# Kinetica-jl/Kinetica.jl

Hardware: AMD Instinct MI355X
Metric: RHS evals/sec (batched sweep) + wall-clock per solve_network, 10k-species CRN (higher is better)
Workload: dtype f64; 1 GPU; synthetic CRN 10000 species / 50000 reactions (seed 12345), batched RHS sweep, B=4096 states per GPU with per-state Arrhenius k (500-1200 K); states_per_gpu=4096, parallelism=replicas x1 (no data-path collective)

## Files before the change

### kinetica_jl_amd/csrc/capi.cpp

```cpp
#include "../../include/kinetica_hip.h"

#include <algorithm>
#include <cmath>
#include <memory>
#include <mutex>
#include <numeric>
#include <string>
#include <cstring>
#include <thread>
#include <vector>

#include "handle.hpp"
#include "lu.hpp"
#include "resident_setup.hpp"
#include "solver.hpp"
#include "solver_kernels.hpp"

using namespace kin;

static thread_local std::string g_create_err;

void kin_network::flush_pending_T(hipStream_t s) {
  if (!k_pending) return;
  launch_arrhenius(host.R, Ea.p, A.p, has_kmax, k_max, t_mult, T_pending, k.p, s);
// ... 1 lines not shown
}

void kin_network::rhs_dev(const double* d_u, double* d_du) {
  if (k_pending) { launch_rates_T(host.R, pending_at(), k.p, d_u, x0.p, x1.p, rate.p, stream); k_pending = false; }
  else launch_rates(host.R, k.p, d_u, x0.p, x1.p, rate.p, stream);
  launch_segsum(rhs_plan.view(), SEG_COEF_SET, rate.p, d_du, SegExtra{}, stream);
}

void kin_network::sweep_dev(int64_t B, const double* d_u, const double* d_k, double* d_du, hipStream_t s) {
  if (!d_k) flush_pending_T(s);
  if (host.N >= 65535) {
    for (int64_t b = 0; b < B; b++) {
      launch_rates(host.R, d_k ? d_k + b * host.R : k.p, d_u + b * host.N, x0.p, x1.p, rate.p, s);
      launch_segsum(rhs_plan.view(), SEG_COEF_SET, rate.p, d_du + b * host.N, SegExtra{}, s);
    }
  } else if (host.big_H > 0) {
    big_scratch.alloc((size_t)std::min<int64_t>(B, n_cu) * (size_t)(host.N - host.big_H + host.n_pairs()));
    launch_sweep_big(n_cu, host.N, host.R, host.n_pairs(), B, host.pairs_adjacent, host.big_H, (int32_t)host.big_tail_ptr.size() - 1,
                     big_rec8.p, big_rec.p, big_expl.p, (int32_t)host.big_expl.size(), sweep_k.p, big_spec.p, big_tptr.p, big_tent.p,
                     big_scratch.p, d_u, d_k, k.p, d_du, host.big_tail_by_species, s);
  } else
    launch_sweep(n_cu, host.N, host.R, host.n_pairs(), B, host.pairs_adjacent, host.pairs_block, sweep_rec.p, sweep_k.p,
                 host.pair_rec64.empty() ? nullptr : sweep_rec64.p, sweep_copy.p, (int)host.sweep_copy_species.size(),
                 host.gen_rec8.empty() ? nullptr : gen_rec8.p, gen_expl.p, (int)host.gen_expl.size(), d_u, d_k, k.p, d_du, s);
}

void kin_network::jac_dev(const double* d_u, double* d_vals) {
  if (k_pending) { launch_drates_T(host.R, pending_at(), k.p, d_u, x0.p, x1.p, dr.p, stream); k_pending = false; }
  else launch_drates(host.R, k.p, d_u, x0.p, x1.p, dr.p, stream);
  launch_segsum(jac_plan.view(), SEG_COEF_SET, dr.p, d_vals, SegExtra{}, stream);
}

#define KIN_TRY(h) try { if (h) KIN_HIP(hipSetDevice((h)->device));
#define KIN_CATCH(h)                                                        \
  }                                                                         \
  catch (const KinError& e) {                                               \
    if (h) (h)->err = e.what(); else g_create_err = e.what();               \
    return e.code;                                                          \
  }                                                                         \
  catch (const std::exception& e) {                                         \
    if (h) (h)->err = e.what(); else g_create_err = e.what();               \
    return KIN_ERR_DEVICE;                                                  \
  }                                                                         \
  return KIN_OK;

static void require(bool c, int code, const char* msg) {
  if (!c) throw KinError(code, msg);
// ... 23 lines not shown

int kin_network_create(int64_t n_species, int64_t n_reactions, const int64_t* reac_ptr, const int64_t* reac_idx,
                       const int64_t* reac_sto, const int64_t* prod_ptr, const int64_t* prod_idx,
                       const int64_t* prod_sto, int index_base, kin_network** out) {
  kin_network* h = nullptr;
  if (!out) { g_create_err = "out is null"; return KIN_ERR_INVALID_ARG; }
  *out = nullptr;
  try {
    NetworkHost H = compile_network(n_species, n_reactions, reac_ptr, reac_idx, reac_sto, prod_ptr, prod_idx,
                                    prod_sto, index_base);
    int ndev = 0;
    if (hipGetDeviceCount(&ndev) != hipSuccess || ndev == 0)
      throw KinError(ERR_DEVICE, "no HIP device available (libkinetica_hip has no CPU fallback)");
    h = new kin_network();
    h->host = std::move(H);
    KIN_HIP(hipGetDevice(&h->device));
    KIN_HIP(hipDeviceGetAttribute(&h->n_cu, hipDeviceAttributeMultiprocessorCount, h->device));
    KIN_HIP(hipStreamCreateWithFlags(&h->stream, hipStreamNonBlocking));
    const NetworkHost& N = h->host;
    hipStream_t s = h->stream;
    h->x0.upload(N.x0, s); h->x1.upload(N.x1, s);
    h->sp_ptr.upload(N.sp_ptr, s); h->sp_rxn.upload(N.sp_rxn, s); h->sp_coef.upload(N.sp_coef, s);
    if (N.N < 65535) { h->sweep_rec.upload(N.pair_rec, s); h->sweep_k.upload(N.pair_k, s); }
    if (!N.gen_rec8.empty()) { h->gen_rec8.upload(N.gen_rec8, s); h->gen_expl.upload(N.gen_expl, s); }
    if (!N.pair_rec64.empty()) { h->sweep_rec64.upload(N.pair_rec64, s); h->sweep_copy.upload(N.sweep_copy_species, s); }
    if (N.big_H > 0) {
      h->big_rec.upload(N.big_rec, s); h->big_rec8.upload(N.big_rec8, s); h->big_expl.upload(N.big_expl, s);
      h->big_spec.upload(N.big_spec_of_label, s);
      h->big_tptr.upload(N.big_tail_ptr, s); h->big_tent.upload(N.big_tail_ent, s);
    }
    h->rhs_plan.upload(build_seg_plan(N.N, N.sp_ptr.data(), nullptr, N.sp_rxn.data(), nullptr, N.sp_coef.data(), false), s);
    h->jac_plan.upload(build_seg_plan(N.nnz(), N.jc_ptr.data(), nullptr, N.jc_src.data(), nullptr, N.jc_coef.data(), false), s);
    h->k.alloc(N.R); h->rate.alloc(N.R); h->dr.alloc(2 * N.R + 2);
    h->u.alloc(N.N); h->du.alloc(N.N); h->jvals.alloc(N.nnz());
    KIN_HIP(hipStreamSynchronize(s));
    *out = h;
  } catch (const KinError& e) {
    g_create_err = e.what();
    delete h;
    return e.code;
  } catch (const std::exception& e) {
    g_create_err = e.what();
    delete h;
    return KIN_ERR_DEVICE;
  }
  return KIN_OK;
}
// ... 552 lines not shown
```

### kinetica_jl_amd/csrc/handle.hpp

```cpp
#pragma once
#include <memory>
#include <string>

#include "common.hpp"
#include "kernels.hpp"
#include "network.hpp"
#include "tiled.hpp"

namespace kin {
struct Solver; struct IntegratorState; struct ResidentSolver; struct EnsembleSolver;
struct ResidentDeleter { void operator()(ResidentSolver* p) const; };
struct EnsembleDeleter { void operator()(EnsembleSolver* p) const; };
}

struct kin_network {
  kin::NetworkHost host;
  hipStream_t stream = nullptr;
  std::string err;

  kin::DevBuf<int32_t> x0, x1, sp_ptr, sp_rxn;
  kin::DevBuf<uint32_t> sweep_rec;
  kin::DevBuf<int32_t> sweep_k;
  kin::DevBuf<uint32_t> sweep_rec64;
  kin::DevBuf<uint32_t> gen_rec8;
  kin::DevBuf<int32_t> gen_expl;
  kin::DevBuf<int32_t> sweep_copy;
  kin::DevBuf<uint32_t> big_rec, big_rec8;
  kin::DevBuf<int32_t> big_spec, big_tptr, big_expl;
  kin::DevBuf<uint32_t> big_tent;
  kin::DevBuf<double> big_scratch;
  kin::DevBuf<float> sp_coef;
  kin::SegPlanDev rhs_plan, jac_plan;

  kin::DevBuf<double> k, Ea, A, table, T_stops;
  bool has_rates = false, has_arrhenius = false, has_kmax = false;
  bool k_pending = false;
  double T_pending = 0.0;
  void set_pending_T(double T) { T_pending = T; k_pending = true; has_rates = true; }
  kin::ArrheniusAt pending_at() const { return kin::ArrheniusAt{Ea.p, A.p, has_kmax ? 1 : 0, k_max, t_mult, T_pending}; }
  void flush_pending_T(hipStream_t s);
  double k_max = 0.0, t_mult = 1.0;
  int64_t table_rows = 0;

  kin::DevBuf<double> u, du, rate, dr, jvals;

  kin::DevBuf<double> b_u, b_k, b_du;

// ... 26 lines not shown
```

### kinetica_jl_amd/csrc/kernels.hip

```cpp
#include "kernels.hpp"

#include "exp_tab.hpp"
#include "segsum_dev.hpp"

#include <algorithm>

namespace kin {

void SegPlanDev::upload(const SegPlanHost& h, hipStream_t s) {
  grp_off.upload(h.grp_off, s); grp_dst.upload(h.grp_dst, s); grp_aux.upload(h.grp_aux, s);
  ell_a.upload(h.ell_a, s); ell_b.upload(h.ell_b, s); ell_c.upload(h.ell_c, s);
  seg_beg.upload(h.seg_beg, s); seg_end.upload(h.seg_end, s); seg_dst.upload(h.seg_dst, s); seg_aux.upload(h.seg_aux, s);
  long_a.upload(h.long_a, s); long_b.upload(h.long_b, s); long_c.upload(h.long_c, s);
  blk_beg.upload(h.blk_beg, s); blk_end.upload(h.blk_end, s); blk_dst.upload(h.blk_dst, s); blk_aux.upload(h.blk_aux, s);
  G = h.n_groups(); S = h.n_segs(); B = h.n_blks(); val_base = h.val_base; ell_total = h.ell_total;
  KIN_HIP(hipStreamSynchronize(s));
}

SegPlanView SegPlanDev::view() const {
  return SegPlanView{grp_off.p, grp_dst.p, grp_aux.p, ell_a.p, ell_b.p, ell_c.p, seg_beg.p, seg_end.p, seg_dst.p, seg_aux.p,
                     blk_beg.p, blk_end.p, blk_dst.p, blk_aux.p, long_a.p, long_b.p, long_c.p, G, S, B, val_base, ell_total};
}

template <int OP, int SEG_WG>
// ... 286 lines not shown
          if (p < P) {
            uint32_t sl[4]; int cf[4];
            const double net = sweep_net<U_IN_LDS>(q[x], kf[x], kr[x], u_s, ub, sl, cf);
#pragma unroll
            for (int j = 0; j < 4; j++) {
              const int sp = (int)sl[j];
              if (sp != 0xffff && sp >= lo && sp < hi)
                __hip_atomic_fetch_add(du_s + (sp - lo), (double)cf[j] * net, __ATOMIC_RELAXED, __HIP_MEMORY_SCOPE_WORKGROUP);
            }
          }
        }
      }
      __syncthreads();
      for (int i = tid * 2; i < hi - lo; i += 2048) {
        if (i + 1 < hi - lo && ((lo & 1) == 0)) *reinterpret_cast<double2*>(dub + lo + i) = *reinterpret_cast<double2*>(du_s + i);
        else { dub[lo + i] = du_s[i]; if (i + 1 < hi - lo) dub[lo + i + 1] = du_s[i + 1]; }
      }
      __syncthreads();
    }
  }
}

constexpr int SWEEP_DUMMY = 64;
__device__ __forceinline__ void sweep_apply(uint2 w, double2 kk, const double* u_s, double* du_s) {
  const uint32_t l0 = w.x & 0x3fffu, l1 = (w.x >> 14) & 0x3fffu, l2 = (w.x >> 28) | ((w.y & 0x3ffu) << 4), l3 = (w.y >> 10) & 0x3fffu;
#if defined(KIN_SWEEP_PROBE) && KIN_SWEEP_PROBE == 1
  const double uf = 1.0 + (double)(l0 + l1), ur = 1.0 + (double)(l2 + l3);
#else
  const double uf = u_s[l0] * u_s[l1], ur = u_s[l2] * u_s[l3];
#endif
  const double net = kk.x * uf - kk.y * ur;
#if defined(KIN_SWEEP_PROBE)
  if (net == 12345.678) du_s[l0] = net;
  return;
#endif
  __hip_atomic_fetch_add(du_s + l0, -net, __ATOMIC_RELAXED, __HIP_MEMORY_SCOPE_WORKGROUP);
  __hip_atomic_fetch_add(du_s + l1, -net, __ATOMIC_RELAXED, __HIP_MEMORY_SCOPE_WORKGROUP);
  __hip_atomic_fetch_add(du_s + l2, net, __ATOMIC_RELAXED, __HIP_MEMORY_SCOPE_WORKGROUP);
  __hip_atomic_fetch_add(du_s + l3, net, __ATOMIC_RELAXED, __HIP_MEMORY_SCOPE_WORKGROUP);
}

template <bool BLK>
__device__ __forceinline__ double2 load_kpair(const double* __restrict__ kb, int p, int P) {
  if (BLK) return make_double2(kb[p], kb[(size_t)P + p]);
  return *reinterpret_cast<const double2*>(kb + 2 * (size_t)p);
}

template <int TR, int ILP, bool BLK, int BS>
__global__ __launch_bounds__(BS) void sweep_reg_kernel(int N, int R, int P, int B, int tile,
                                                         const uint2* __restrict__ rec64, const int32_t* __restrict__ copy_species,
                                                         int n_copy, const double* __restrict__ u,
                                                         const double* __restrict__ k_b, const double* __restrict__ k_1,
                                                         double* __restrict__ du) {
  extern __shared__ double lds[];
  double* du_s = lds;
  double* u_s = lds + tile;
  const int tid = threadIdx.x;
  constexpr int UPT = 5;
  const uint64_t dl = (uint64_t)N + (uint64_t)(tid & 63);
  const uint64_t ew = dl | (dl << 14) | (dl << 28) | (dl << 42);
  const uint2 EMPTY = {(uint32_t)ew, (uint32_t)(ew >> 32)};
  if (tid < SWEEP_DUMMY) { u_s[N + tid] = 1.0; du_s[N + tid] = 0.0; }
  const int csp = tid < n_copy ? copy_species[min(tid, max(n_copy - 1, 0))] : -1;
  if (csp >= 0) du_s[N + SWEEP_DUMMY + tid] = 0.0;
  const int Pm1 = P - 1, Bm1 = B - 1, csp_c = max(csp, 0);
  uint2 rc[TR > 0 ? TR : 1];
#pragma unroll
  for (int i = 0; i < TR; i++) {
    const int p = tid + i * BS;
    const uint2 w = rec64[min(p, Pm1)];
    rc[i].x = p < P ? w.x : EMPTY.x;
    rc[i].y = p < P ? w.y : EMPTY.y;
  }
  double2 un[UPT];
  int b = blockIdx.x;
  {
    const double* ub = u + (size_t)min(b, Bm1) * N;
#pragma unroll
    for (int x = 0; x < UPT; x++) {
      const double2 t = *reinterpret_cast<const double2*>(ub + min((tid + x * BS) * 2, N - 2));
      un[x].x = t.x; un[x].y = t.y;
    }
  }
  for (int i = tid * 2; i < N; i += (2 * BS)) *reinterpret_cast<double2*>(du_s + i) = make_double2(0.0, 0.0);
  double ucn = u[(size_t)min(b, Bm1) * N + csp_c];
  constexpr bool KPRE = TR >= ILP;
  double2 k0[KPRE ? ILP : 1];
  if (KPRE) {
    const double* kb = k_b ? k_b + (size_t)min(b, Bm1) * R : k_1;
#pragma unroll
    for (int x = 0; x < ILP; x++) k0[x] = load_kpair<BLK>(kb, min(tid + x * BS, Pm1), P);
  }
  for (; b < B; b += gridDim.x) {
    const double* kb = k_b ? k_b + (size_t)b * R : k_1;
    double* dub = du + (size_t)b * N;
#pragma unroll
    for (int x = 0; x < UPT; x++) {
      const int i = (tid + x * BS) * 2;
      if (i < N) *reinterpret_cast<double2*>(u_s + i) = un[x];
    }
    if (csp >= 0) u_s[N + SWEEP_DUMMY + tid] = ucn;
    __syncthreads();
    const int bn = b + gridDim.x;
    ucn = u[(size_t)min(bn, Bm1) * N + csp_c];
    {
      const double* ub = u + (size_t)min(bn, Bm1) * N;
#pragma unroll
      for (int x = 0; x < UPT; x++) {
        const double2 t = *reinterpret_cast<const double2*>(ub + min((tid + x * BS) * 2, N - 2));
        un[x].x = t.x; un[x].y = t.y;
      }
    }
#pragma unroll
    for (int i0 = 0; i0 < TR; i0 += ILP) {
      double2 kk[ILP];
#pragma unroll
      for (int x = 0; x < ILP; x++) {
        if (KPRE && i0 == 0) kk[x] = k0[x];
        else kk[x] = load_kpair<BLK>(kb, min(tid + (i0 + x) * BS, Pm1), P);
      }
#pragma unroll
      for (int x = 0; x < ILP; x++) {
        uint2 w = rc[i0 + x];
        asm volatile("" : "+v"(w.x), "+v"(w.y));
        sweep_apply(w, kk[x], u_s, du_s);
      }
    }
    for (int p0 = tid + TR * BS; p0 < P; p0 += BS * ILP) {
      double2 kk[ILP];
      uint2 w[ILP];
#pragma unroll
      for (int x = 0; x < ILP; x++) {
        const int p = p0 + x * BS;
        const bool ok = p < P;
        kk[x] = load_kpair<BLK>(kb, min(p, Pm1), P);
        const uint2 q = rec64[min(p, Pm1)];
        w[x].x = ok ? q.x : EMPTY.x;
        w[x].y = ok ? q.y : EMPTY.y;
      }
#pragma unroll
      for (int x = 0; x < ILP; x++) sweep_apply(w[x], kk[x], u_s, du_s);
    }
    if (KPRE) {
      const double* kn = k_b ? k_b + (size_t)min(bn, Bm1) * R : k_1;
#pragma unroll
      for (int x = 0; x < ILP; x++) k0[x] = load_kpair<BLK>(kn, min(tid + x * BS, Pm1), P);
    }
    __syncthreads();
    if (n_copy > 0) {
      if (csp >= 0) {
        const double v = du_s[N + SWEEP_DUMMY + tid];
        du_s[N + SWEEP_DUMMY + tid] = 0.0;
        __hip_atomic_fetch_add(du_s + csp, v, __ATOMIC_RELAXED, __HIP_MEMORY_SCOPE_WORKGROUP);
      }
      __syncthreads();
    }
    for (int i = tid * 2; i < N; i += (2 * BS)) {
      *reinterpret_cast<double2*>(dub + i) = *reinterpret_cast<double2*>(du_s + i);
      *reinterpret_cast<double2*>(du_s + i) = make_double2(0.0, 0.0);
    }
  }
}

template <int TR, int ILP, bool BLK, int BS>
static void launch_sweep_reg_t(int grid, size_t smem, int N, int R, int P, int B, int tile, const void* rec64,
                               const int32_t* copy_species, int n_copy, const double* u, const double* k_b, const double* k_1,
                               double* du, hipStream_t s) {
  KIN_HIP(hipFuncSetAttribute((const void*)sweep_reg_kernel<TR, ILP, BLK, BS>, hipFuncAttributeMaxDynamicSharedMemorySize, 160 * 1024));
  hipLaunchKernelGGL((sweep_reg_kernel<TR, ILP, BLK, BS>), dim3(grid), dim3(BS), smem, s, N, R, P, B, tile, (const uint2*)rec64,
                     copy_species, n_copy, u, k_b, k_1, du);
}

template <int BS>
__global__ __launch_bounds__(BS) void sweep_gen_kernel(int N, int R, int P, int B, int tile, const uint2* __restrict__ rec8,
                                                         const int2* __restrict__ pair_k, const SweepRec* __restrict__ rec,
                                                         const int32_t* __restrict__ expl, int n_expl,
                                                         const double* __restrict__ u, const double* __restrict__ k_b,
                                                         const double* __restrict__ k_1, double* __restrict__ du) {
  extern __shared__ double lds[];
  double* du_s = lds;
  double* u_s = lds + tile;
  const int tid = threadIdx.x;
  constexpr int ILP = 4;
  const uint32_t dl = (uint32_t)(N + (tid & 63));
  const uint2 EMPTY = {dl | (dl << 16), dl | (dl << 16)};
  if (tid < SWEEP_DUMMY) { u_s[N + tid] = 1.0; du_s[N + tid] = 0.0; }
  for (int i = tid; i < N; i += BS) du_s[i] = 0.0;
  constexpr int UPT = 10;
  double un[UPT];
  int b = blockIdx.x;
#pragma unroll
  for (int x = 0; x < UPT; x++) { const int i = tid + x * BS; un[x] = (b < B && i < N) ? u[(size_t)b * N + i] : 0.0; }
  for (; b < B; b += gridDim.x) {
    const double* kb = k_b ? k_b + (size_t)b * R : k_1;
    double* dub = du + (size_t)b * N;
#pragma unroll
    for (int x = 0; x < UPT; x++) { const int i = tid + x * BS; if (i < N) u_s[i] = un[x]; }
    __syncthreads();
    const int bn = b + gridDim.x;
#pragma unroll
    for (int x = 0; x < UPT; x++) { const int i = tid + x * BS; un[x] = (bn < B && i < N) ? u[(size_t)bn * N + i] : 0.0; }
    for (int qq = tid; qq < P; qq += BS * ILP) {
      uint2 w[ILP];
      int2 ki[ILP];
      double kf[ILP], kr[ILP];
#pragma unroll
      for (int x = 0; x < ILP; x++) {
        const int p = qq + x * BS;
        w[x] = p < P ? rec8[p] : EMPTY;
        ki[x] = p < P ? pair_k[p] : make_int2(-1, -1);
      }
#pragma unroll
      for (int x = 0; x < ILP; x++) {
        kf[x] = ki[x].x >= 0 ? kb[ki[x].x] : 0.0;
        kr[x] = ki[x].y >= 0 ? kb[ki[x].y] : 0.0;
      }
#pragma unroll
      for (int x = 0; x < ILP; x++) {
        const uint32_t l0 = w[x].x & 0xffffu, l1 = w[x].x >> 16, l2 = w[x].y & 0xffffu, l3 = w[x].y >> 16;
#if defined(KIN_SWEEP_PROBE)
        const double net = KIN_SWEEP_PROBE == 1 ? kf[x] * (1.0 + (double)(l0 + l1)) - kr[x] * (1.0 + (double)(l2 + l3))
                                                : kf[x] * (u_s[l0] * u_s[l1]) - kr[x] * (u_s[l2] * u_s[l3]);
        if (net == 12345.678) du_s[l0] = net;
        continue;
#else
        const double net = kf[x] * (u_s[l0] * u_s[l1]) - kr[x] * (u_s[l2] * u_s[l3]);
#endif
        __hip_atomic_fetch_add(du_s + l0, -net, __ATOMIC_RELAXED, __HIP_MEMORY_SCOPE_WORKGROUP);
        __hip_atomic_fetch_add(du_s + l1, -net, __ATOMIC_RELAXED, __HIP_MEMORY_SCOPE_WORKGROUP);
        __hip_atomic_fetch_add(du_s + l2, net, __ATOMIC_RELAXED, __HIP_MEMORY_SCOPE_WORKGROUP);
        __hip_atomic_fetch_add(du_s + l3, net, __ATOMIC_RELAXED, __HIP_MEMORY_SCOPE_WORKGROUP);
      }
    }
    for (int i = tid; i < n_expl; i += BS) {
      const int p = expl[i];
      const SweepRec q = rec[p];
      const uint32_t a = q.ops & 0xffffu, c = q.ops >> 16;
      double net = kb[pair_k[p].x] * u_s[a];
      if (c != 0xffffu) net *= u_s[c];
      const uint32_t sl[4] = {q.s01 & 0xffffu, q.s01 >> 16, q.s23 & 0xffffu, q.s23 >> 16};
#pragma unroll
      for (int j = 0; j < 4; j++)
        if (sl[j] != 0xffffu)
          __hip_atomic_fetch_add(du_s + sl[j], (double)(int)(int8_t)((uint32_t)q.coef >> (8 * j)) * net, __ATOMIC_RELAXED,
                                 __HIP_MEMORY_SCOPE_WORKGROUP);
    }
    __syncthreads();
    for (int i = tid; i < N; i += BS) { dub[i] = du_s[i]; du_s[i] = 0.0; }
  }
}

template <bool ADJ>
__global__ __launch_bounds__(1024) void sweep_big_kernel(int N, int R, int P, int B, int H, int n_tail_tiles,
                                                         const uint2* __restrict__ rec8, const SweepRec* __restrict__ rec,
                                                         const int32_t* __restrict__ expl, int n_expl,
// ... 144 lines not shown
}

void launch_sweep_big(int n_cu, int64_t N, int64_t R, int64_t P, int64_t B, bool adjacent, int32_t H, int32_t n_tail_tiles, const void* rec8,
                      const void* rec, const int32_t* expl, int32_t n_expl, const void* pair_k, const int32_t* spec_of_label,
                      const int32_t* tail_ptr, const void* tail_ent, double* scratch, const double* u, const double* k_b,
                      const double* k_1, double* du, bool tail_by_species, hipStream_t s) {
  if (B == 0) return;
  const int grid = (int)std::min<int64_t>(B, n_cu);
  const bool adj = adjacent && ((((uintptr_t)(k_b ? k_b : k_1)) & 15) == 0);
  if (adj) launch_sweep_big_t<true>(grid, (int)N, (int)R, (int)P, (int)B, H, n_tail_tiles, rec8, rec, expl, n_expl, pair_k, spec_of_label, tail_ptr, tail_ent, scratch, u, k_b, k_1, du, tail_by_species ? 1 : 0, s);
  else launch_sweep_big_t<false>(grid, (int)N, (int)R, (int)P, (int)B, H, n_tail_tiles, rec8, rec, expl, n_expl, pair_k, spec_of_label, tail_ptr, tail_ent, scratch, u, k_b, k_1, du, tail_by_species ? 1 : 0, s);
  KIN_HIP(hipGetLastError());
}

template <bool U_IN_LDS, bool ADJ>
static void launch_sweep_t(int grid, size_t smem, int N, int R, int P, int B, int tile, int n_tiles, const void* rec,
                           const void* pair_k, const double* u, const double* k_b, const double* k_1, double* du, hipStream_t s) {
  KIN_HIP(hipFuncSetAttribute((const void*)sweep_lds_kernel<U_IN_LDS, ADJ>, hipFuncAttributeMaxDynamicSharedMemorySize, 160 * 1024));
  hipLaunchKernelGGL((sweep_lds_kernel<U_IN_LDS, ADJ>), dim3(grid), dim3(1024), smem, s, N, R, P, B, tile, n_tiles,
                     (const SweepRec*)rec, (const int2*)pair_k, u, k_b, k_1, du);
}

void launch_sweep(int n_cu, int64_t N, int64_t R, int64_t P, int64_t B, bool adjacent, bool block, const void* rec, const void* pair_k,
                  const void* rec64, const int32_t* copy_species, int n_copy, const void* gen_rec8, const int32_t* gen_expl,
                  int n_gen_expl, const double* u, const double* k_b, const double* k_1, double* du, hipStream_t s) {
  if (B == 0) return;
  const size_t lds_max = 160 * 1024;
  const int grid = (int)std::min<int64_t>(B, n_cu);
  const bool adj = adjacent && ((((uintptr_t)(k_b ? k_b : k_1)) & 15) == 0);
  if ((size_t)(2 * N) * 8 <= lds_max) {
    const int tile = (int)((N + 1) / 2 * 2);
    const size_t smem = (size_t)(tile + N) * 8;
    constexpr int use_reg = 8;
    if ((adj || block) && rec64 && use_reg >= 0 && ((((uintptr_t)u) | ((uintptr_t)du)) & 15) == 0 && N % 2 == 0 &&
        (size_t)(2 * (N + SWEEP_DUMMY + n_copy)) * 8 <= lds_max && n_copy <= 1024) {
      const int rtile = (int)N + SWEEP_DUMMY + n_copy + (n_copy & 1);
      const size_t rsmem = (size_t)2 * rtile * 8;
      const int bs = (N <= 2560 && n_copy <= 256) ? 256 : ((N <= 5120 && n_copy <= 512) ? 512 : 1024);
      const int per_cu = (int)std::max<size_t>(1, std::min<size_t>(2048 / bs, lds_max / rsmem));
      const int rgrid = (int)std::min<int64_t>(B, (int64_t)n_cu * per_cu);
      const int64_t Tr = P / bs;
#define KIN_REG_ARGS rgrid, rsmem, (int)N, (int)R, (int)P, (int)B, rtile, rec64, copy_species, n_copy, u, k_b, k_1, du, s
#define KIN_REG_GO(TT, II)                                                                   \
  do {                                                                                       \
    if (bs == 256) { if (adj) launch_sweep_reg_t<TT, II, false, 256>(KIN_REG_ARGS); else launch_sweep_reg_t<TT, II, true, 256>(KIN_REG_ARGS); }   \
    else if (bs == 512) { if (adj) launch_sweep_reg_t<TT, II, false, 512>(KIN_REG_ARGS); else launch_sweep_reg_t<TT, II, true, 512>(KIN_REG_ARGS); } \
    else { if (adj) launch_sweep_reg_t<TT, II, false, 1024>(KIN_REG_ARGS); else launch_sweep_reg_t<TT, II, true, 1024>(KIN_REG_ARGS); }       \
  } while (0)
      const int want = (int)std::min<int64_t>(use_reg, Tr);
      if (want >= 16) KIN_REG_GO(16, 4);
      else if (want >= 12) KIN_REG_GO(12, 4);
      else if (want >= 8) KIN_REG_GO(8, 4);
      else if (want >= 4) KIN_REG_GO(4, 4);
      else if (use_reg == 1) KIN_REG_GO(0, 8);
      else KIN_REG_GO(0, 4);
#undef KIN_REG_GO
#undef KIN_REG_ARGS
      KIN_HIP(hipGetLastError());
      return;
    }
    if (gen_rec8 && (size_t)(2 * (N + SWEEP_DUMMY)) * 8 <= lds_max) {
      const int gtile = (int)N + SWEEP_DUMMY;
      const size_t gsmem = (size_t)2 * gtile * 8;
      const int bs = N <= 2560 ? 256 : (N <= 5120 ? 512 : 1024);
      const int per_cu = (int)std::max<size_t>(1, std::min<size_t>(2048 / bs, lds_max / gsmem));
      const int ggrid = (int)std::min<int64_t>(B, (int64_t)n_cu * per_cu);
#define KIN_GEN_GO(BSZ)                                                                                                                 \
  do {                                                                                                                                  \
    KIN_HIP(hipFuncSetAttribute((const void*)sweep_gen_kernel<BSZ>, hipFuncAttributeMaxDynamicSharedMemorySize, 160 * 1024));           \
    hipLaunchKernelGGL(sweep_gen_kernel<BSZ>, dim3(ggrid), dim3(BSZ), gsmem, s, (int)N, (int)R, (int)P, (int)B, gtile,                  \
                       (const uint2*)gen_rec8, (const int2*)pair_k, (const SweepRec*)rec, gen_expl, n_gen_expl, u, k_b, k_1, du);       \
  } while (0)
      if (bs == 256) KIN_GEN_GO(256);
      else if (bs == 512) KIN_GEN_GO(512);
      else KIN_GEN_GO(1024);
#undef KIN_GEN_GO
      KIN_HIP(hipGetLastError());
      return;
    }
    if (adj) launch_sweep_t<true, true>(grid, smem, (int)N, (int)R, (int)P, (int)B, tile, 1, rec, pair_k, u, k_b, k_1, du, s);
    else launch_sweep_t<true, false>(grid, smem, (int)N, (int)R, (int)P, (int)B, tile, 1, rec, pair_k, u, k_b, k_1, du, s);
  } else {
    const int tile = 16 * 1024;
    const int n_tiles = (int)ceil_div(N, tile);
    if (adj) launch_sweep_t<false, true>(grid, (size_t)tile * 8, (int)N, (int)R, (int)P, (int)B, tile, n_tiles, rec, pair_k, u, k_b, k_1, du, s);
    else launch_sweep_t<false, false>(grid, (size_t)tile * 8, (int)N, (int)R, (int)P, (int)B, tile, n_tiles, rec, pair_k, u, k_b, k_1, du, s);
  }
  KIN_HIP(hipGetLastError());
}

}
```

### kinetica_jl_amd/csrc/kernels.hpp

```cpp
#pragma once
#include "common.hpp"
#include "network.hpp"

namespace kin {

struct SegPlanView {
  const int32_t* grp_off; const int32_t* grp_dst; const int32_t* grp_aux;
  const int32_t* ell_a; const int32_t* ell_b; const float* ell_c;
  const int32_t* seg_beg; const int32_t* seg_end; const int32_t* seg_dst; const int32_t* seg_aux;
  const int32_t* blk_beg; const int32_t* blk_end; const int32_t* blk_dst; const int32_t* blk_aux;
  const int32_t* long_a; const int32_t* long_b; const float* long_c;
  int32_t G, S, B;
  int32_t val_base, ell_total;
};

struct SegPlanDev {
  DevBuf<int32_t> grp_off, grp_dst, grp_aux, ell_a, ell_b, seg_beg, seg_end, seg_dst, seg_aux, blk_beg, blk_end, blk_dst, blk_aux, long_a, long_b;
  DevBuf<float> ell_c, long_c;
  int32_t G = 0, S = 0, B = 0, val_base = -1, ell_total = 0;
  void upload(const SegPlanHost& h, hipStream_t s);
  SegPlanView view() const;
};

enum SegOp : int {
// ... 4 lines not shown
  SEG_PROD_AUXSUB = 4,
  SEG_PROD_SET = 5,
  SEG_PROD_NEG = 6,
};
struct SegExtra {
  const double* psi = nullptr; const double* d = nullptr; double cscal = 0.0;
  const int* skip = nullptr;
};

void launch_segsum(const SegPlanView& p, SegOp op, const double* src, double* out, const SegExtra& ex, hipStream_t s);

void launch_rates(int64_t R, const double* k, const double* u, const int32_t* x0, const int32_t* x1, double* rate, hipStream_t s);
void launch_drates(int64_t R, const double* k, const double* u, const int32_t* x0, const int32_t* x1, double* dr, hipStream_t s);

struct ArrheniusAt { const double* Ea; const double* A; int has_kmax; double k_max, t_mult, T; };
void launch_rates_T(int64_t R, const ArrheniusAt& at, double* k, const double* u, const int32_t* x0, const int32_t* x1, double* rate, hipStream_t s);
void launch_drates_T(int64_t R, const ArrheniusAt& at, double* k, const double* u, const int32_t* x0, const int32_t* x1, double* dr, hipStream_t s);

void launch_arrhenius(int64_t n, const double* Ea, const double* A, int has_kmax, double k_max, double t_mult, double T, double* k, hipStream_t s);
void launch_rate_table(int64_t n, int64_t n_stops, const double* Ea, const double* A, int has_kmax, double k_max,
                       double t_mult, const double* T, double* table, hipStream_t s);

void launch_sweep(int n_cu, int64_t N, int64_t R, int64_t P, int64_t B, bool adjacent, bool block, const void* rec, const void* pair_k,
                  const void* rec64, const int32_t* copy_species, int n_copy, const void* gen_rec8, const int32_t* gen_expl,
                  int n_gen_expl, const double* u, const double* k_b, const double* k_1, double* du, hipStream_t s);

void launch_sweep_big(int n_cu, int64_t N, int64_t R, int64_t P, int64_t B, bool adjacent, int32_t H, int32_t n_tail_tiles, const void* rec8,
                      const void* rec, const int32_t* expl, int32_t n_expl, const void* pair_k, const int32_t* spec_of_label,
                      const int32_t* tail_ptr, const void* tail_ent, double* scratch, const double* u, const double* k_b,
                      const double* k_1, double* du, bool tail_by_species, hipStream_t s);

}
```

### kinetica_jl_amd/csrc/network.cpp

```cpp
#include "network.hpp"

#include <algorithm>
#include <map>
#include <numeric>
#include <string>

namespace kin {

SegPlanHost build_seg_plan(int64_t n_rows, const int32_t* ptr, const int32_t* dst, const int32_t* a,
                           const int32_t* b, const float* c, bool skip_empty, const int32_t* aux,
                           std::vector<int32_t>* slot_of_entry) {
  SegPlanHost P;
  const bool prod = b != nullptr;
  if (slot_of_entry) slot_of_entry->assign((size_t)ptr[n_rows], -1);
  std::vector<int32_t> shorts, longs;
  for (int64_t i = 0; i < n_rows; i++) {
    int32_t len = ptr[i + 1] - ptr[i];
    if (len == 0 && skip_empty) continue;
    (len <= SegPlanHost::SHORT_MAX ? shorts : longs).push_back((int32_t)i);
  }
  {
    std::vector<size_t> start(SegPlanHost::SHORT_MAX + 2, 0);
    for (int32_t r : shorts) start[ptr[r + 1] - ptr[r] + 1]++;
    for (size_t l = 1; l < start.size(); l++) start[l] += start[l - 1];
// ... 214 lines not shown
        const int K = (int)std::max<int64_t>(0, std::min<int64_t>(32, spare / 7));
        std::vector<int64_t> refs(N, 0);
        for (int64_t q = 0; q < 4 * P; q++) if (inst[q] < N) refs[inst[q]]++;
        std::vector<int32_t> order(N);
        std::iota(order.begin(), order.end(), 0);
        std::stable_sort(order.begin(), order.end(), [&](int32_t x, int32_t y) { return refs[x] > refs[y]; });
        std::vector<int32_t> rank_of(N, -1);
        H.sweep_copy_species.clear();
        for (int r = 0; r < K && r < N && refs[order[r]] >= 64; r++) {
          rank_of[order[r]] = r;
          for (int c = 1; c < 8; c++) H.sweep_copy_species.push_back(order[r]);
        }
        for (int64_t p = 0; p < P; p++) {
          uint64_t f[4];
          for (int j = 0; j < 4; j++) {
            const int32_t sp = inst[4 * p + j];
            const int c = (int)(p & 7);
            f[j] = (sp < N && rank_of[sp] >= 0 && c > 0) ? (uint64_t)(N + 64 + rank_of[sp] * 7 + (c - 1)) : (uint64_t)sp;
          }
          const uint64_t w = f[0] | (f[1] << 14) | (f[2] << 28) | (f[3] << 42);
          H.pair_rec64.push_back((uint32_t)w);
          H.pair_rec64.push_back((uint32_t)(w >> 32));
        }
      }
    }
    if (!H.pairs_adjacent && !H.pairs_block && (size_t)(N + 64) * 16 <= 160 * 1024) {
      const int64_t P = H.n_pairs();
      for (int64_t p = 0; p < P; p++) {
        const uint32_t s01 = H.pair_rec[4 * p], s23 = H.pair_rec[4 * p + 1], co = H.pair_rec[4 * p + 2], ops = H.pair_rec[4 * p + 3];
        const uint32_t sl[4] = {s01 & 0xffffu, s01 >> 16, s23 & 0xffffu, s23 >> 16};
        const uint32_t dummy = (uint32_t)N + (uint32_t)(p & 63);
        uint32_t side[2][2] = {{dummy, dummy}, {dummy, dummy}};
        int cnt[2] = {0, 0};
        if (ops == 0xffffffffu) {
          for (int j = 0; j < 4; j++) {
            if (sl[j] == 0xffffu) continue;
            const int c = (int)(int8_t)(co >> (8 * j));
            const int sd = c < 0 ? 0 : 1;
            for (int q = 0; q < (c < 0 ? -c : c) && cnt[sd] < 2; q++) side[sd][cnt[sd]++] = sl[j];
          }
        } else {
          H.gen_expl.push_back((int32_t)p);
        }
        H.gen_rec8.push_back(side[0][0] | (side[0][1] << 16));
        H.gen_rec8.push_back(side[1][0] | (side[1][1] << 16));
      }
    }
    if ((size_t)N * 16 > 160 * 1024 && N + 64 < 65535) {
      const int64_t P = H.n_pairs();
      const int32_t Hh = 10000;
      std::vector<int64_t> cnt(N, 0);
      for (int64_t p = 0; p < P; p++) {
        const uint32_t s01 = H.pair_rec[4 * p], s23 = H.pair_rec[4 * p + 1];
        const uint32_t sl[4] = {s01 & 0xffffu, s01 >> 16, s23 & 0xffffu, s23 >> 16};
        for (int j = 0; j < 4; j++) if (sl[j] != 0xffffu) cnt[sl[j]]++;
        const uint32_t ops = H.pair_rec[4 * p + 3];
        if (ops != 0xffffffffu) { cnt[ops & 0xffffu]++; if ((ops >> 16) != 0xffffu) cnt[ops >> 16]++; }
      }
      std::vector<int32_t> order(N);
      std::iota(order.begin(), order.end(), 0);
      std::stable_sort(order.begin(), order.end(), [&](int32_t a, int32_t b) { return cnt[a] > cnt[b]; });
      std::vector<char> is_hub(N, 0);
      for (int32_t q = 0; q < Hh; q++) is_hub[order[q]] = 1;
      std::vector<int32_t> label(N);
      H.big_spec_of_label.clear();
      for (int32_t sp = 0; sp < N; sp++) if (is_hub[sp]) { label[sp] = (int32_t)H.big_spec_of_label.size(); H.big_spec_of_label.push_back(sp); }
      for (int32_t sp = 0; sp < N; sp++) if (!is_hub[sp]) { label[sp] = (int32_t)H.big_spec_of_label.size(); H.big_spec_of_label.push_back(sp); }
      H.big_H = Hh;
// ... 79 lines not shown
```

### kinetica_jl_amd/csrc/network.hpp

```cpp
#pragma once
#include <cstdint>
#include <vector>

#include "common.hpp"

namespace kin {

struct SegPlanHost {
  static constexpr int SHORT_MAX = 8;
  static constexpr int SEG_LEN = 256;
  static constexpr int BLK_PASS = 12288;
  std::vector<int32_t> grp_off;
  std::vector<int32_t> grp_dst;
  std::vector<int32_t> grp_aux;
  std::vector<int32_t> ell_a, ell_b;
  std::vector<float> ell_c;
  std::vector<int32_t> seg_beg, seg_end;
  std::vector<int32_t> seg_dst;
  std::vector<int32_t> seg_aux;
  std::vector<int32_t> blk_beg, blk_end, blk_dst, blk_aux;
  std::vector<int32_t> long_a, long_b;
  std::vector<float> long_c;
  int32_t val_base = -1;
  int32_t ell_total = 0, long_total = 0;
  int32_t n_groups() const { return (int32_t)grp_off.size() - 1; }
  int32_t n_segs() const { return (int32_t)seg_beg.size(); }
  int32_t n_blks() const { return (int32_t)blk_beg.size(); }
};

SegPlanHost build_seg_plan(int64_t n_rows, const int32_t* ptr, const int32_t* dst, const int32_t* a,
                           const int32_t* b, const float* c, bool skip_empty, const int32_t* aux = nullptr,
                           std::vector<int32_t>* slot_of_entry = nullptr);

struct NetworkHost {
  int64_t N = 0, R = 0;
  std::vector<int32_t> x0, x1;
  std::vector<int32_t> y0, y1;
  bool products_le2 = true;
  std::vector<int32_t> slot_sp;
  std::vector<int32_t> slot_co;
  std::vector<uint32_t> pair_rec;
  std::vector<int32_t> pair_k;
  std::vector<uint32_t> gen_rec8;
  std::vector<int32_t> gen_expl;
  std::vector<int32_t> sweep_copy_species;
  std::vector<uint32_t> pair_rec64;
  int32_t big_H = 0;
  bool big_tail_by_species = false;
  std::vector<int32_t> big_spec_of_label;
  std::vector<uint32_t> big_rec;
  std::vector<uint32_t> big_rec8;
  std::vector<int32_t> big_expl;
  std::vector<int32_t> big_tail_ptr;
  std::vector<uint32_t> big_tail_ent;
  bool pairs_adjacent = false;
  bool pairs_block = false;
  int64_t n_pairs() const { return (int64_t)pair_k.size() / 2; }
  std::vector<int32_t> sp_ptr, sp_rxn;
  std::vector<float> sp_coef;
  std::vector<int32_t> j_ptr, j_col, j_diag;
  std::vector<int32_t> jc_ptr, jc_src;
  std::vector<float> jc_coef;
  int64_t nnz() const { return (int64_t)j_col.size(); }
};

NetworkHost compile_network(int64_t n_species, int64_t n_reactions, const int64_t* reac_ptr,
// ... 5 lines not shown
```

Measured before the change: 9.419 million RHS evals/s.

## Pad sweep record arrays and restructure streaming loop with nontemporal loads

Pads the 64-bit and generic pair-record arrays (and a new gen_k copy) with dummy entries so that the sweep kernels can drop per-element bounds checks and empty-record selects. The streaming tail of the register-resident sweep is replaced by a host-precomputed count of ILP and ILP+1 batches, using nontemporal loads for rate constants and nontemporal stores for the output. It also prefetches more k pairs and fixes TR/ILP selection to a compile-time ILP. Sched barriers are added in both kernels to control instruction interleaving. The trade-off is extra device memory for the padding and higher register pressure from the larger prefetch.

```diff
diff --git a/kinetica_jl_amd/csrc/capi.cpp b/kinetica_jl_amd/csrc/capi.cpp
--- a/kinetica_jl_amd/csrc/capi.cpp
+++ b/kinetica_jl_amd/csrc/capi.cpp
@@ -47,7 +47,7 @@
   } else
     launch_sweep(n_cu, host.N, host.R, host.n_pairs(), B, host.pairs_adjacent, host.pairs_block, sweep_rec.p, sweep_k.p,
                  host.pair_rec64.empty() ? nullptr : sweep_rec64.p, sweep_copy.p, (int)host.sweep_copy_species.size(),
-                 host.gen_rec8.empty() ? nullptr : gen_rec8.p, gen_expl.p, (int)host.gen_expl.size(), d_u, d_k, k.p, d_du, s);
+                 host.gen_rec8.empty() ? nullptr : gen_rec8.p, gen_k.p, gen_expl.p, (int)host.gen_expl.size(), d_u, d_k, k.p, d_du, s);
 }
 
 void kin_network::jac_dev(const double* d_u, double* d_vals) {
@@ -117,7 +117,7 @@
     h->x0.upload(N.x0, s); h->x1.upload(N.x1, s);
     h->sp_ptr.upload(N.sp_ptr, s); h->sp_rxn.upload(N.sp_rxn, s); h->sp_coef.upload(N.sp_coef, s);
     if (N.N < 65535) { h->sweep_rec.upload(N.pair_rec, s); h->sweep_k.upload(N.pair_k, s); }
-    if (!N.gen_rec8.empty()) { h->gen_rec8.upload(N.gen_rec8, s); h->gen_expl.upload(N.gen_expl, s); }
+    if (!N.gen_rec8.empty()) { h->gen_rec8.upload(N.gen_rec8, s); h->gen_k.upload(N.gen_k, s); h->gen_expl.upload(N.gen_expl, s); }
     if (!N.pair_rec64.empty()) { h->sweep_rec64.upload(N.pair_rec64, s); h->sweep_copy.upload(N.sweep_copy_species, s); }
     if (N.big_H > 0) {
       h->big_rec.upload(N.big_rec, s); h->big_rec8.upload(N.big_rec8, s); h->big_expl.upload(N.big_expl, s);
diff --git a/kinetica_jl_amd/csrc/handle.hpp b/kinetica_jl_amd/csrc/handle.hpp
--- a/kinetica_jl_amd/csrc/handle.hpp
+++ b/kinetica_jl_amd/csrc/handle.hpp
@@ -23,6 +23,7 @@
   kin::DevBuf<int32_t> sweep_k;
   kin::DevBuf<uint32_t> sweep_rec64;
   kin::DevBuf<uint32_t> gen_rec8;
+  kin::DevBuf<int32_t> gen_k;
   kin::DevBuf<int32_t> gen_expl;
   kin::DevBuf<int32_t> sweep_copy;
   kin::DevBuf<uint32_t> big_rec, big_rec8;
diff --git a/kinetica_jl_amd/csrc/kernels.hip b/kinetica_jl_amd/csrc/kernels.hip
--- a/kinetica_jl_amd/csrc/kernels.hip
+++ b/kinetica_jl_amd/csrc/kernels.hip
@@ -332,6 +332,9 @@
 }
 
 constexpr int SWEEP_DUMMY = 64;
+#ifndef KIN_SWEEP_ILP
+#define KIN_SWEEP_ILP 4
+#endif
 __device__ __forceinline__ void sweep_apply(uint2 w, double2 kk, const double* u_s, double* du_s) {
   const uint32_t l0 = w.x & 0x3fffu, l1 = (w.x >> 14) & 0x3fffu, l2 = (w.x >> 28) | ((w.y & 0x3ffu) << 4), l3 = (w.y >> 10) & 0x3fffu;
 #if defined(KIN_SWEEP_PROBE) && KIN_SWEEP_PROBE == 1
@@ -350,14 +353,46 @@
   __hip_atomic_fetch_add(du_s + l3, net, __ATOMIC_RELAXED, __HIP_MEMORY_SCOPE_WORKGROUP);
 }
 
+typedef double kin_d2 __attribute__((ext_vector_type(2)));
 template <bool BLK>
 __device__ __forceinline__ double2 load_kpair(const double* __restrict__ kb, int p, int P) {
-  if (BLK) return make_double2(kb[p], kb[(size_t)P + p]);
-  return *reinterpret_cast<const double2*>(kb + 2 * (size_t)p);
+  const char* base = reinterpret_cast<const char*>(kb);
+  if (BLK) return make_double2(__builtin_nontemporal_load(reinterpret_cast<const double*>(base + (uint32_t)p * 8u)),
+                               __builtin_nontemporal_load(reinterpret_cast<const double*>(base + ((uint32_t)P + (uint32_t)p) * 8u)));
+  const kin_d2 v = __builtin_nontemporal_load(reinterpret_cast<const kin_d2*>(base + (uint32_t)p * 16u));
+  return make_double2(v.x, v.y);
+}
+__device__ __forceinline__ uint2 load_rec64(const uint2* __restrict__ rec64, int p) {
+  return *reinterpret_cast<const uint2*>(reinterpret_cast<const char*>(rec64) + (uint32_t)p * 8u);
+}
+
+template <int NB, bool BLK, int BS>
+__device__ __forceinline__ void sweep_stream_batch(const double* __restrict__ kb, const uint2* __restrict__ rec64, int p0, int Pm1,
+                                                   int P, const double* u_s, double* du_s) {
+  double2 kk[NB];
+  uint2 w[NB];
+#pragma unroll
+  for (int x = 0; x < NB; x++) {
+    const int p = p0 + x * BS;
+    w[x] = load_rec64(rec64, p);
+    kk[x] = load_kpair<BLK>(kb, min(p, Pm1), P);
+    __builtin_amdgcn_sched_barrier(0);
+  }
+#pragma unroll
+  for (int x = 0; x < NB; x++) sweep_apply(w[x], kk[x], u_s, du_s);
+  __builtin_amdgcn_sched_barrier(0);
+}
+
+struct SweepStreamPlan { int n_a, n_b; };
+static SweepStreamPlan sweep_stream_plan(int64_t P, int bs, int tr, int ilp) {
+  const int64_t rows = ceil_div(P, (int64_t)bs), S = std::max<int64_t>(0, rows - tr);
+  const int64_t rounds = ceil_div(S, (int64_t)(ilp + 1));
+  const int64_t n_b = std::max<int64_t>(0, S - ilp * rounds);
+  return {(int)(rounds - n_b), (int)n_b};
 }
 
 template <int TR, int ILP, bool BLK, int BS>
-__global__ __launch_bounds__(BS) void sweep_reg_kernel(int N, int R, int P, int B, int tile,
+__global__ __launch_bounds__(BS) void sweep_reg_kernel(int N, int R, int P, int B, int tile, int n_a, int n_b,
                                                          const uint2* __restrict__ rec64, const int32_t* __restrict__ copy_species,
                                                          int n_copy, const double* __restrict__ u,
                                                          const double* __restrict__ k_b, const double* __restrict__ k_1,
@@ -367,21 +402,13 @@
   double* u_s = lds + tile;
   const int tid = threadIdx.x;
   constexpr int UPT = 5;
-  const uint64_t dl = (uint64_t)N + (uint64_t)(tid & 63);
-  const uint64_t ew = dl | (dl << 14) | (dl << 28) | (dl << 42);
-  const uint2 EMPTY = {(uint32_t)ew, (uint32_t)(ew >> 32)};
   if (tid < SWEEP_DUMMY) { u_s[N + tid] = 1.0; du_s[N + tid] = 0.0; }
   const int csp = tid < n_copy ? copy_species[min(tid, max(n_copy - 1, 0))] : -1;
   if (csp >= 0) du_s[N + SWEEP_DUMMY + tid] = 0.0;
   const int Pm1 = P - 1, Bm1 = B - 1, csp_c = max(csp, 0);
   uint2 rc[TR > 0 ? TR : 1];
 #pragma unroll
-  for (int i = 0; i < TR; i++) {
-    const int p = tid + i * BS;
-    const uint2 w = rec64[min(p, Pm1)];
-    rc[i].x = p < P ? w.x : EMPTY.x;
-    rc[i].y = p < P ? w.y : EMPTY.y;
-  }
+  for (int i = 0; i < TR; i++) rc[i] = rec64[tid + i * BS];
   double2 un[UPT];
   int b = blockIdx.x;
   {
@@ -395,11 +422,12 @@
   for (int i = tid * 2; i < N; i += (2 * BS)) *reinterpret_cast<double2*>(du_s + i) = make_double2(0.0, 0.0);
   double ucn = u[(size_t)min(b, Bm1) * N + csp_c];
   constexpr bool KPRE = TR >= ILP;
-  double2 k0[KPRE ? ILP : 1];
+  constexpr int KP = TR >= 2 * ILP ? 2 * ILP : ILP;
+  double2 k0[KPRE ? KP : 1];
   if (KPRE) {
     const double* kb = k_b ? k_b + (size_t)min(b, Bm1) * R : k_1;
 #pragma unroll
-    for (int x = 0; x < ILP; x++) k0[x] = load_kpair<BLK>(kb, min(tid + x * BS, Pm1), P);
+    for (int x = 0; x < KP; x++) k0[x] = load_kpair<BLK>(kb, min(tid + x * BS, Pm1), P);
   }
   for (; b < B; b += gridDim.x) {
     const double* kb = k_b ? k_b + (size_t)b * R : k_1;
@@ -421,13 +449,15 @@
         un[x].x = t.x; un[x].y = t.y;
       }
     }
+    int tl = tid;
+    asm volatile("" : "+v"(tl));
 #pragma unroll
     for (int i0 = 0; i0 < TR; i0 += ILP) {
       double2 kk[ILP];
 #pragma unroll
       for (int x = 0; x < ILP; x++) {
-        if (KPRE && i0 == 0) kk[x] = k0[x];
-        else kk[x] = load_kpair<BLK>(kb, min(tid + (i0 + x) * BS, Pm1), P);
+        if (KPRE && i0 + x < KP) kk[x] = k0[i0 + x];
+        else kk[x] = load_kpair<BLK>(kb, min(tl + (i0 + x) * BS, Pm1), P);
       }
 #pragma unroll
       for (int x = 0; x < ILP; x++) {
@@ -436,25 +466,15 @@
         sweep_apply(w, kk[x], u_s, du_s);
       }
     }
-    for (int p0 = tid + TR * BS; p0 < P; p0 += BS * ILP) {
-      double2 kk[ILP];
-      uint2 w[ILP];
-#pragma unroll
-      for (int x = 0; x < ILP; x++) {
-        const int p = p0 + x * BS;
-        const bool ok = p < P;
-        kk[x] = load_kpair<BLK>(kb, min(p, Pm1), P);
-        const uint2 q = rec64[min(p, Pm1)];
-        w[x].x = ok ? q.x : EMPTY.x;
-        w[x].y = ok ? q.y : EMPTY.y;
-      }
-#pragma unroll
-      for (int x = 0; x < ILP; x++) sweep_apply(w[x], kk[x], u_s, du_s);
+    {
+      int p0 = tl + TR * BS;
+      for (int r = 0; r < n_a; r++, p0 += BS * ILP) sweep_stream_batch<ILP, BLK, BS>(kb, rec64, p0, Pm1, P, u_s, du_s);
+      for (int r = 0; r < n_b; r++, p0 += BS * (ILP + 1)) sweep_stream_batch<ILP + 1, BLK, BS>(kb, rec64, p0, Pm1, P, u_s, du_s);
     }
     if (KPRE) {
       const double* kn = k_b ? k_b + (size_t)min(bn, Bm1) * R : k_1;
 #pragma unroll
-      for (int x = 0; x < ILP; x++) k0[x] = load_kpair<BLK>(kn, min(tid + x * BS, Pm1), P);
+      for (int x = 0; x < KP; x++) k0[x] = load_kpair<BLK>(kn, min(tl + x * BS, Pm1), P);
     }
     __syncthreads();
     if (n_copy > 0) {
@@ -465,9 +485,20 @@
       }
       __syncthreads();
     }
-    for (int i = tid * 2; i < N; i += (2 * BS)) {
-      *reinterpret_cast<double2*>(dub + i) = *reinterpret_cast<double2*>(du_s + i);
-      *reinterpret_cast<double2*>(du_s + i) = make_double2(0.0, 0.0);
+    {
+      double2 v[UPT];
+#pragma unroll
+      for (int x = 0; x < UPT; x++) v[x] = *reinterpret_cast<double2*>(du_s + min((tid + x * BS) * 2, N - 2));
+#pragma unroll
+      for (int x = 0; x < UPT; x++) {
+        const int i = (tid + x * BS) * 2;
+        if (i < N) {
+          kin_d2 t;
+          t.x = v[x].x; t.y = v[x].y;
+          __builtin_nontemporal_store(t, reinterpret_cast<kin_d2*>(dub + i));
+          *reinterpret_cast<double2*>(du_s + i) = make_double2(0.0, 0.0);
+        }
+      }
     }
   }
 }
@@ -477,13 +508,16 @@
                                const int32_t* copy_species, int n_copy, const double* u, const double* k_b, const double* k_1,
                                double* du, hipStream_t s) {
   KIN_HIP(hipFuncSetAttribute((const void*)sweep_reg_kernel<TR, ILP, BLK, BS>, hipFuncAttributeMaxDynamicSharedMemorySize, 160 * 1024));
-  hipLaunchKernelGGL((sweep_reg_kernel<TR, ILP, BLK, BS>), dim3(grid), dim3(BS), smem, s, N, R, P, B, tile, (const uint2*)rec64,
-                     copy_species, n_copy, u, k_b, k_1, du);
+  const SweepStreamPlan plan = sweep_stream_plan(P, BS, TR, ILP);
+  static_assert(2 * ILP <= SWEEP_REC_PAD / 1024, "a batch that starts in the last row must stay inside the padded record array");
+  hipLaunchKernelGGL((sweep_reg_kernel<TR, ILP, BLK, BS>), dim3(grid), dim3(BS), smem, s, N, R, P, B, tile, plan.n_a, plan.n_b,
+                     (const uint2*)rec64, copy_species, n_copy, u, k_b, k_1, du);
 }
 
 template <int BS>
 __global__ __launch_bounds__(BS) void sweep_gen_kernel(int N, int R, int P, int B, int tile, const uint2* __restrict__ rec8,
-                                                         const int2* __restrict__ pair_k, const SweepRec* __restrict__ rec,
+                                                         const int2* __restrict__ gen_k, const int2* __restrict__ pair_k,
+                                                         const SweepRec* __restrict__ rec,
                                                          const int32_t* __restrict__ expl, int n_expl,
                                                          const double* __restrict__ u, const double* __restrict__ k_b,
                                                          const double* __restrict__ k_1, double* __restrict__ du) {
@@ -492,15 +526,13 @@
   double* u_s = lds + tile;
   const int tid = threadIdx.x;
   constexpr int ILP = 4;
-  const uint32_t dl = (uint32_t)(N + (tid & 63));
-  const uint2 EMPTY = {dl | (dl << 16), dl | (dl << 16)};
   if (tid < SWEEP_DUMMY) { u_s[N + tid] = 1.0; du_s[N + tid] = 0.0; }
   for (int i = tid; i < N; i += BS) du_s[i] = 0.0;
   constexpr int UPT = 10;
   double un[UPT];
   int b = blockIdx.x;
 #pragma unroll
-  for (int x = 0; x < UPT; x++) { const int i = tid + x * BS; un[x] = (b < B && i < N) ? u[(size_t)b * N + i] : 0.0; }
+  for (int x = 0; x < UPT; x++) un[x] = u[(size_t)min(b, B - 1) * N + min(tid + x * BS, N - 1)];
   for (; b < B; b += gridDim.x) {
     const double* kb = k_b ? k_b + (size_t)b * R : k_1;
     double* dub = du + (size_t)b * N;
@@ -509,7 +541,7 @@
     __syncthreads();
     const int bn = b + gridDim.x;
 #pragma unroll
-    for (int x = 0; x < UPT; x++) { const int i = tid + x * BS; un[x] = (bn < B && i < N) ? u[(size_t)bn * N + i] : 0.0; }
+    for (int x = 0; x < UPT; x++) un[x] = u[(size_t)min(bn, B - 1) * N + min(tid + x * BS, N - 1)];
     for (int qq = tid; qq < P; qq += BS * ILP) {
       uint2 w[ILP];
       int2 ki[ILP];
@@ -517,14 +549,18 @@
 #pragma unroll
       for (int x = 0; x < ILP; x++) {
         const int p = qq + x * BS;
-        w[x] = p < P ? rec8[p] : EMPTY;
-        ki[x] = p < P ? pair_k[p] : make_int2(-1, -1);
-      }
+        w[x] = rec8[p];
+        ki[x] = gen_k[p];
+      }
+      __builtin_amdgcn_sched_barrier(0);
 #pragma unroll
       for (int x = 0; x < ILP; x++) {
-        kf[x] = ki[x].x >= 0 ? kb[ki[x].x] : 0.0;
-        kr[x] = ki[x].y >= 0 ? kb[ki[x].y] : 0.0;
-      }
+        kf[x] = kb[ki[x].x];
+        kr[x] = kb[max(ki[x].y, 0)];
+      }
+      __builtin_amdgcn_sched_barrier(0);
+#pragma unroll
+      for (int x = 0; x < ILP; x++) kr[x] = ki[x].y >= 0 ? kr[x] : 0.0;
 #pragma unroll
       for (int x = 0; x < ILP; x++) {
         const uint32_t l0 = w[x].x & 0xffffu, l1 = w[x].x >> 16, l2 = w[x].y & 0xffffu, l3 = w[x].y >> 16;
@@ -541,6 +577,7 @@
         __hip_atomic_fetch_add(du_s + l2, net, __ATOMIC_RELAXED, __HIP_MEMORY_SCOPE_WORKGROUP);
         __hip_atomic_fetch_add(du_s + l3, net, __ATOMIC_RELAXED, __HIP_MEMORY_SCOPE_WORKGROUP);
       }
+      __builtin_amdgcn_sched_barrier(0);
     }
     for (int i = tid; i < n_expl; i += BS) {
       const int p = expl[i];
@@ -731,8 +768,9 @@
 }
 
 void launch_sweep(int n_cu, int64_t N, int64_t R, int64_t P, int64_t B, bool adjacent, bool block, const void* rec, const void* pair_k,
-                  const void* rec64, const int32_t* copy_species, int n_copy, const void* gen_rec8, const int32_t* gen_expl,
-                  int n_gen_expl, const double* u, const double* k_b, const double* k_1, double* du, hipStream_t s) {
+                  const void* rec64, const int32_t* copy_species, int n_copy, const void* gen_rec8, const void* gen_k,
+                  const int32_t* gen_expl, int n_gen_expl, const double* u, const double* k_b, const double* k_1, double* du,
+                  hipStream_t s) {
   if (B == 0) return;
   const size_t lds_max = 160 * 1024;
   const int grid = (int)std::min<int64_t>(B, n_cu);
@@ -740,8 +778,7 @@
   if ((size_t)(2 * N) * 8 <= lds_max) {
     const int tile = (int)((N + 1) / 2 * 2);
     const size_t smem = (size_t)(tile + N) * 8;
-    constexpr int use_reg = 8;
-    if ((adj || block) && rec64 && use_reg >= 0 && ((((uintptr_t)u) | ((uintptr_t)du)) & 15) == 0 && N % 2 == 0 &&
+    if ((adj || block) && rec64 && R < ((int64_t)1 << 29) && ((((uintptr_t)u) | ((uintptr_t)du)) & 15) == 0 && N % 2 == 0 &&
         (size_t)(2 * (N + SWEEP_DUMMY + n_copy)) * 8 <= lds_max && n_copy <= 1024) {
       const int rtile = (int)N + SWEEP_DUMMY + n_copy + (n_copy & 1);
       const size_t rsmem = (size_t)2 * rtile * 8;
@@ -756,13 +793,10 @@
     else if (bs == 512) { if (adj) launch_sweep_reg_t<TT, II, false, 512>(KIN_REG_ARGS); else launch_sweep_reg_t<TT, II, true, 512>(KIN_REG_ARGS); } \
     else { if (adj) launch_sweep_reg_t<TT, II, false, 1024>(KIN_REG_ARGS); else launch_sweep_reg_t<TT, II, true, 1024>(KIN_REG_ARGS); }       \
   } while (0)
-      const int want = (int)std::min<int64_t>(use_reg, Tr);
-      if (want >= 16) KIN_REG_GO(16, 4);
-      else if (want >= 12) KIN_REG_GO(12, 4);
-      else if (want >= 8) KIN_REG_GO(8, 4);
-      else if (want >= 4) KIN_REG_GO(4, 4);
-      else if (use_reg == 1) KIN_REG_GO(0, 8);
-      else KIN_REG_GO(0, 4);
+      constexpr int I = KIN_SWEEP_ILP;
+      if (Tr >= 2 * I) KIN_REG_GO(2 * I, I);
+      else if (Tr >= I) KIN_REG_GO(I, I);
+      else KIN_REG_GO(0, I);
 #undef KIN_REG_GO
 #undef KIN_REG_ARGS
       KIN_HIP(hipGetLastError());
@@ -778,7 +812,8 @@
   do {                                                                                                                                  \
     KIN_HIP(hipFuncSetAttribute((const void*)sweep_gen_kernel<BSZ>, hipFuncAttributeMaxDynamicSharedMemorySize, 160 * 1024));           \
     hipLaunchKernelGGL(sweep_gen_kernel<BSZ>, dim3(ggrid), dim3(BSZ), gsmem, s, (int)N, (int)R, (int)P, (int)B, gtile,                  \
-                       (const uint2*)gen_rec8, (const int2*)pair_k, (const SweepRec*)rec, gen_expl, n_gen_expl, u, k_b, k_1, du);       \
+                       (const uint2*)gen_rec8, (const int2*)gen_k, (const int2*)pair_k, (const SweepRec*)rec, gen_expl, n_gen_expl,     \
+                       u, k_b, k_1, du);                                                                                                \
   } while (0)
       if (bs == 256) KIN_GEN_GO(256);
       else if (bs == 512) KIN_GEN_GO(512);
diff --git a/kinetica_jl_amd/csrc/kernels.hpp b/kinetica_jl_amd/csrc/kernels.hpp
--- a/kinetica_jl_amd/csrc/kernels.hpp
+++ b/kinetica_jl_amd/csrc/kernels.hpp
@@ -50,8 +50,9 @@
                        double t_mult, const double* T, double* table, hipStream_t s);
 
 void launch_sweep(int n_cu, int64_t N, int64_t R, int64_t P, int64_t B, bool adjacent, bool block, const void* rec, const void* pair_k,
-                  const void* rec64, const int32_t* copy_species, int n_copy, const void* gen_rec8, const int32_t* gen_expl,
-                  int n_gen_expl, const double* u, const double* k_b, const double* k_1, double* du, hipStream_t s);
+                  const void* rec64, const int32_t* copy_species, int n_copy, const void* gen_rec8, const void* gen_k,
+                  const int32_t* gen_expl, int n_gen_expl, const double* u, const double* k_b, const double* k_1, double* du,
+                  hipStream_t s);
 
 void launch_sweep_big(int n_cu, int64_t N, int64_t R, int64_t P, int64_t B, bool adjacent, int32_t H, int32_t n_tail_tiles, const void* rec8,
                       const void* rec, const int32_t* expl, int32_t n_expl, const void* pair_k, const int32_t* spec_of_label,
diff --git a/kinetica_jl_amd/csrc/network.cpp b/kinetica_jl_amd/csrc/network.cpp
--- a/kinetica_jl_amd/csrc/network.cpp
+++ b/kinetica_jl_amd/csrc/network.cpp
@@ -260,6 +260,12 @@
           H.pair_rec64.push_back((uint32_t)w);
           H.pair_rec64.push_back((uint32_t)(w >> 32));
         }
+        for (int64_t p = P; P > 0 && p < P + SWEEP_REC_PAD; p++) {
+          const uint64_t d = (uint64_t)N + (uint64_t)(p & 63);
+          const uint64_t w = d | (d << 14) | (d << 28) | (d << 42);
+          H.pair_rec64.push_back((uint32_t)w);
+          H.pair_rec64.push_back((uint32_t)(w >> 32));
+        }
       }
     }
     if (!H.pairs_adjacent && !H.pairs_block && (size_t)(N + 64) * 16 <= 160 * 1024) {
@@ -282,6 +288,14 @@
         }
         H.gen_rec8.push_back(side[0][0] | (side[0][1] << 16));
         H.gen_rec8.push_back(side[1][0] | (side[1][1] << 16));
+      }
+      H.gen_k = H.pair_k;
+      for (int64_t p = P; P > 0 && p < P + SWEEP_REC_PAD; p++) {
+        const uint32_t d = (uint32_t)N + (uint32_t)(p & 63);
+        H.gen_rec8.push_back(d | (d << 16));
+        H.gen_rec8.push_back(d | (d << 16));
+        H.gen_k.push_back(0);
+        H.gen_k.push_back(-1);
       }
     }
     if ((size_t)N * 16 > 160 * 1024 && N + 64 < 65535) {
diff --git a/kinetica_jl_amd/csrc/network.hpp b/kinetica_jl_amd/csrc/network.hpp
--- a/kinetica_jl_amd/csrc/network.hpp
+++ b/kinetica_jl_amd/csrc/network.hpp
@@ -32,6 +32,8 @@
                            const int32_t* b, const float* c, bool skip_empty, const int32_t* aux = nullptr,
                            std::vector<int32_t>* slot_of_entry = nullptr);
 
+constexpr int64_t SWEEP_REC_PAD = 16 * 1024;
+
 struct NetworkHost {
   int64_t N = 0, R = 0;
   std::vector<int32_t> x0, x1;
@@ -42,6 +44,7 @@
   std::vector<uint32_t> pair_rec;
   std::vector<int32_t> pair_k;
   std::vector<uint32_t> gen_rec8;
+  std::vector<int32_t> gen_k;
   std::vector<int32_t> gen_expl;
   std::vector<int32_t> sweep_copy_species;
   std::vector<uint32_t> pair_rec64;
```

Result: faster. 10.24 million RHS evals/s (median of 6 runs) (+8.7%).
